# TritonDataCenter/containerpilot

Hardware: NVIDIA H100
Metric: events/sec through Bus.Publish (deliveries/s = 32-byte records landed in subscriber mailboxes) (higher is better)
Workload: dtype u8

## Files before the change

containerpilot_b200/_native.py:

```python
from __future__ import annotations

import ctypes as C
import os

import numpy as np

HERE = os.path.dirname(os.path.abspath(__file__))
LIB_PATH = os.environ.get("CPBUS_LIB") or os.path.join(HERE, "libcpbus.so")

N_CODES = 17
MASK_ALL = 0x0001FFFF
TARGET_ALL = 0xFFFFFFFF
F_TICK, F_UNICAST = 0x1, 0x2
CFG_LOSSLESS, CFG_DIGEST, CFG_SPARSE_TICKS, CFG_SPARSE_RECORDS = 0x1, 0x2, 0x4, 0x8
CFG_DROP_MISSED_TICKS = 0x10
STORE_AUTO, STORE_V4, STORE_V8, STORE_BULK = 0, 1, 2, 3

OK, EINVAL, ENOMEM, ECUDA, EAGAIN, ENOSPC, ENOENT, ECLOSED, ENODEV, EORDER, ETIMEDOUT = 0, -1, -2, -3, -4, -5, -6, -7, -8, -9, -10
PUT_STAMP, PUT_RAW, PUT_NOWAIT = 0, 1, 2
EPHEMERAL_BIT, EPHEMERAL_SLOTS = 0x80000000, 65536
DUE_CLOCK, DUE_ARM, DUE_ONESHOT, DUE_DISARM, DUE_UNSUB, DUE_LAUNCH = 0, 1, 2, 3, 4, 5
DUE_CATCHUP = 6


# ... 83 lines not shown
    "cpbus_stream_set_timeout": (C.c_int, [C.c_void_p, C.c_uint32]),
    "cpbus_stream_close": (C.c_int, [C.c_void_p]),
    "cpbus_shared_alloc": (C.c_int, [C.c_void_p, C.c_size_t, _P(C.c_void_p), C.c_char_p]),
    "cpbus_shared_open": (C.c_int, [C.c_void_p, C.c_char_p, _P(C.c_void_p)]),
    "cpbus_shared_close": (C.c_int, [C.c_void_p, C.c_void_p]),
    "cpbus_drain": (C.c_int, [C.c_void_p, C.c_uint32, C.c_void_p, C.c_size_t, _P(C.c_size_t), _P(C.c_uint64)]),
    "cpbus_drain_many": (C.c_int, [C.c_void_p, C.c_uint32, C.c_uint32, C.c_void_p, C.c_size_t, C.c_void_p, C.c_void_p, _P(C.c_size_t)]),
    "cpbus_drain_ready": (C.c_int, [C.c_void_p, C.c_uint32, C.c_uint32, C.c_uint32, C.c_void_p, C.c_size_t, C.c_void_p,
                                    C.c_size_t, _P(C.c_size_t), _P(C.c_size_t), _P(C.c_uint32)]),
    "cpbus_lagging": (C.c_int, [C.c_void_p, C.c_uint32, C.c_uint32, C.c_uint32, C.c_uint32, C.c_void_p, C.c_size_t,
                                _P(C.c_size_t), _P(C.c_uint32), _P(LagSummary)]),
    "cpbus_blockers": (C.c_int, [C.c_void_p, C.c_void_p, C.c_size_t, _P(C.c_size_t)]),
    "cpbus_stream_blockers": (C.c_int, [C.c_void_p, C.c_void_p, C.c_size_t, _P(C.c_size_t)]),
    "cpbus_consume_all": (C.c_int, [C.c_void_p]),
    "cpbus_peek_window": (C.c_int, [C.c_void_p, C.c_uint32, C.c_void_p, C.c_size_t, _P(C.c_size_t)]),
    "cpbus_digest": (C.c_int, [C.c_void_p, C.c_uint32, C.c_uint32, C.c_void_p]),
    "cpbus_digest_fold": (C.c_int, [C.c_void_p, C.c_uint32, C.c_uint32, _P(C.c_uint64 * 4)]),
    "cpbus_digest_fold_begin": (C.c_int, [C.c_void_p, C.c_uint32, C.c_uint32, _P(C.c_uint32)]),
    "cpbus_digest_fold_end": (C.c_int, [C.c_void_p, C.c_uint32, _P(C.c_uint64 * 4)]),
    "cpbus_step_result_begin": (C.c_int, [C.c_void_p, _P(C.c_uint32)]),
    "cpbus_step_result_end": (C.c_int, [C.c_void_p, C.c_uint32, _P(C.c_uint64 * 4)]),
    "cpbus_debug_events": (C.c_int, [C.c_void_p, C.c_void_p, C.c_size_t, _P(C.c_size_t)]),
    "cpbus_stats": (C.c_int, [C.c_void_p, _P(Stats)]),
    "cpbus_publish_counts": (C.c_int, [C.c_void_p, C.c_void_p, C.c_size_t, _P(C.c_size_t)]),
    "cpbus_device_ptrs": (C.c_int, [C.c_void_p, _P(C.c_void_p), _P(C.c_void_p)]),
    "cpbus_code_name": (C.c_char_p, [C.c_int]),
    "cpbus_code_from_string": (C.c_int, [C.c_char_p]),
    "cpbus_strerror": (C.c_char_p, [C.c_int]),
    "cpbus_last_cuda_error": (C.c_char_p, []),
    "cpbus_abi_version": (C.c_uint32, []),
    "cpbus_split_plan": (C.c_int, [C.c_void_p, C.c_size_t, C.c_uint32, C.c_uint64, C.c_uint64, C.c_uint64, C.c_void_p, C.c_void_p, C.c_size_t, _P(C.c_size_t)]),
    "cpbus_mask_order": (C.c_size_t, [C.c_void_p, C.c_void_p, C.c_uint32, C.c_uint32, C.c_uint32, C.c_int, C.c_void_p]),
    "cpbus_due_trace": (C.c_int, [C.c_void_p, C.c_size_t, C.c_uint32, C.c_uint32, C.c_void_p, C.c_size_t, _P(C.c_size_t)]),
    "cpbus_sparse_plan": (C.c_int, [C.c_void_p, C.c_void_p, C.c_uint32, C.c_void_p, C.c_void_p, C.c_uint32, C.c_void_p,
                                    C.c_size_t, C.c_void_p, C.c_size_t, C.c_uint32, C.c_size_t, C.c_size_t, C.c_void_p,
                                    C.c_size_t, C.c_void_p, C.c_size_t, _P(C.c_size_t), _P(C.c_size_t)]),
    "cpbus_record_hash": (C.c_uint64, [_P(Event)]),
    "cpbus_digest_multiplier": (C.c_uint64, []),
}
GROUP_CALLS = ("intern", "intern_ephemeral", "source", "subscribe", "subscribe_many", "subscribe_pairs", "subscribe_pairs_many",
               "unsubscribe", "set_mask", "timer_add", "timer_add_many", "timer_cancel", "publish", "send", "advance", "flush",
               "sync", "drain", "drain_ready", "lagging", "blockers", "consume_all", "peek_window", "digest", "digest_fold",
               "debug_events", "stats", "publish_counts")
SYMBOLS["cpbus_group_create"] = (C.c_int, [_P(Config), C.c_void_p, C.c_uint32, _P(C.c_void_p)])
SYMBOLS["cpbus_group_destroy"] = (C.c_int, [C.c_void_p])
SYMBOLS.update({f"cpbus_group_{name}": SYMBOLS[f"cpbus_{name}"] for name in GROUP_CALLS})
# ... 34 lines not shown
```

containerpilot_b200/csrc/cpbus.cu:

```cuda
#include "cpbus_kernels.cuh"

#include <algorithm>
#include <chrono>
#include <cstdio>
#include <cstdlib>
#include <cstring>
#include <deque>
#include <map>
#include <mutex>
#include <new>
#include <string>
#include <thread>
#include <unordered_map>
#include <vector>

using namespace cpbus_dev;

namespace {

thread_local char g_cuda_err[256] = "";

#define CK(call)                                                                                   \
  do {                                                                                             \
    cudaError_t e_ = (call);                                                                       \
// ... 362 lines not shown
  static constexpr int kStage = 8;
  static constexpr int kDevSlots = 64, kDevEpoch = 16;
  cpbus_event* d_stage = nullptr;
  cudaEvent_t epoch_done[kDevSlots / kDevEpoch] = {};
  uint32_t dev_slot = 0;
  cpbus_event* h_batch[kStage] = {};
  cudaEvent_t h2d_done[kStage] = {};
  cudaStream_t copy_stream = nullptr;
  cudaStream_t result_stream = nullptr;
  DevResultSlot* d_result = nullptr;
  DevResultSlot* h_result = nullptr;
  cudaEvent_t result_done[8] = {};
  uint32_t result_next = 0;
  DevStats* h_stats = nullptr;
  unsigned long long* h_fold = nullptr;
  int cur = 0;

  std::vector<uint32_t> h_mask;
  std::vector<uint8_t> h_active;
  std::vector<uint8_t> h_npairs;
  uint2* d_pairs = nullptr;
  uint32_t n_paired = 0;
  uint32_t* d_order = nullptr;
  uint32_t n_order = 0, n_filtered = 0;
  bool order_dirty = true;
  uint32_t n_next = 0, n_active = 0;

  uint64_t room_lb = 0;

  bool sparse = false, sparse_records = false;
  DueIndex due;
  std::vector<uint32_t> due_slots;
  SubIndex rec_index;
  std::vector<cpbus_plan_entry> plan;
  std::vector<uint32_t> plan_idx;
  std::vector<uint64_t> plan_pairs;
  unsigned char* h_plan = nullptr; unsigned char* d_plan = nullptr; size_t plan_bytes_cap = 0;
  cudaEvent_t plan_done = nullptr;
  cudaEvent_t records_done = nullptr;
  std::vector<uint32_t> catchup_slots;
  uint32_t* d_catchup = nullptr; size_t catchup_cap = 0;

  std::unordered_map<std::string, uint32_t> intern;
  std::vector<std::string> sources;
  size_t intern_bytes = 0;
  struct EphSlot { std::string s; uint32_t gen = 0; bool live = false; };
// ... 103 lines not shown
    for (size_t k = 1; k < count.size(); k++) count[k] += count[k - 1];
    const size_t base = order.size();
    order.resize(base + count.back());
    for (uint32_t i = lo; i < hi; i++) if (!active || active[i]) order[base + count[masks[i] & CPBUS_MASK_ALL]++] = i;
    if (heavy_first) {
      const size_t nb = order.size() - base;
      uint32_t pc_count[34] = {};
      for (size_t k = 0; k < nb; k++) pc_count[32 - __builtin_popcount(masks[order[base + k]] & CPBUS_MASK_ALL) + 1]++;
      for (int k = 1; k < 34; k++) pc_count[k] += pc_count[k - 1];
      tmp.resize(nb);
      for (size_t k = 0; k < nb; k++) tmp[pc_count[32 - __builtin_popcount(masks[order[base + k]] & CPBUS_MASK_ALL)]++] = order[base + k];
      std::copy(tmp.begin(), tmp.end(), order.begin() + base);
    }
  }
}

int rebuild_order(cpbus* b) {
  std::vector<uint32_t> order;
  static_assert(sizeof(b->h_active[0]) == 1, "h_active is a byte vector");
  mask_order(b->h_mask.data(), reinterpret_cast<const uint8_t*>(b->h_active.data()), b->n_next, b->R, b->order_block, true, order);
  b->n_order = (uint32_t)order.size();
  if (b->n_order) {
    CK(cudaMemcpyAsync(b->d_order, order.data(), (size_t)b->n_order * 4, cudaMemcpyHostToDevice, b->stream));
    CK(cudaStreamSynchronize(b->stream));
  }
  b->order_dirty = false;
  return CPBUS_OK;
}

constexpr int kFanoutMaxSmem = 200 * 1024;

enum { kLaunchPlain = 0, kLaunchFollow = 1, kLaunchRound = 2 };

template <int STORE, bool TIMERS, bool DIGEST, bool ORDERED, bool PAIRS = false>
int launch_fanout_t(cpbus* b, const FanoutParams& p, uint32_t grid, size_t smem, int kind) {
  static bool attr_done[3][64] = {};
  void (*kernel)(FanoutParams) = kind == kLaunchRound  ? fanout_round_kernel<STORE, TIMERS, DIGEST, ORDERED, PAIRS>
                               : kind == kLaunchFollow ? fanout_follow_kernel<STORE, TIMERS, DIGEST, ORDERED, PAIRS>
                                                       : fanout_kernel<STORE, TIMERS, DIGEST, ORDERED, PAIRS>;
  const int dev = b->device & 63;
  if (!attr_done[kind][dev]) {
    CK(cudaFuncSetAttribute(kernel, cudaFuncAttributeMaxDynamicSharedMemorySize, kFanoutMaxSmem));
    attr_done[kind][dev] = true;
  }
  cudaLaunchConfig_t cfg{};
  cfg.gridDim = dim3(grid); cfg.blockDim = dim3(kThreads); cfg.dynamicSmemBytes = smem; cfg.stream = b->stream;
// ... 90 lines not shown
  if (follow) {
    p.follow_clock = b->d_follow_clock; p.follow_rec = sa->follow_rec; p.follow_window = max_window(b);
    p.follow_from_host = sa->follow_from_host ? 1u : 0u;
  }
  p.prefetch_src = o.pf_src; p.prefetch_dst = o.pf_dst; p.prefetch_n = o.pf_n;
  p.batch_dep = o.batch_dep ? 1u : 0u; p.n_ev = n;
  p.n_subs = b->n_next; p.ring_cap = b->R; p.K = b->K; p.sub_base = b->cfg.sub_id_base;
  p.use_digest = b->use_digest; p.lossless = b->lossless; p.timers_on = b->n_timers > 0 && b->K > 0;
  p.smem_cap = (n + 31u) & ~31u;
  const size_t hot_bytes = (size_t)b->n_next * (sizeof(SubCtl) + (p.timers_on ? b->K * sizeof(DevTimer) : 0));
  p.hints = b->hints >= 0 ? (uint32_t)b->hints : (hot_bytes <= (64u << 20) ? 1u : 0u);
  const uint32_t need = (b->n_next + kWarpsPerCta - 1) / kWarpsPerCta;
  uint32_t grid = b->cfg.grid_ctas ? std::max(1u, std::min(b->cfg.grid_ctas, need)) : 0u;
  int rc;
  const bool pairs_on = b->n_paired > 0 && b->d_pairs;
  p.pairs = pairs_on ? b->d_pairs : nullptr;
  size_t smem = fanout_smem_bytes(p.smem_cap) + (pairs_on ? kPairFilterBytes : 0);
  if (!pairs_on && !p.timers_on && b->n_filtered > 0) {
    if (b->order_dirty) { const int rc_order = rebuild_order(b); if (rc_order) return rc_order; }
    if (b->n_order) {
      const uint32_t scale = std::max(1u, (p.n_ev + 128u) / 256u);
      uint32_t spw = b->subs_per_warp ? std::min(32u, b->subs_per_warp)
                                      : std::max(4u, std::min(16u / scale, b->n_order / (20480u * scale)));
      p.order = b->d_order; p.n_order = b->n_order; p.spw = spw;
      const uint32_t warps = (b->n_order + spw - 1) / spw;
      grid = std::max(1u, (warps + kWarpsPerCta - 1) / kWarpsPerCta);
    }
  }
  if (pairs_on && !b->cfg.grid_ctas) {
    const uint32_t blocks = (b->n_next + 31u) / 32u;
    grid = std::max(1u, std::min((blocks + kWarpsPerCta - 1) / kWarpsPerCta, (uint32_t)b->sm_count * 16u));
  }
  if (!pairs_on && !p.order) {
    uint32_t spw = b->subs_per_warp;
    if (grid) spw = std::max(1u, (need + grid - 1) / grid);
    else if (!spw) {
      const uint32_t scale = std::max(1u, (p.n_ev + 128u) / 256u);
      const uint32_t cap = std::max(1u, 16u / scale);
      spw = std::max(1u, std::min(cap, (need + (uint32_t)b->sm_count * 7 * scale) / ((uint32_t)b->sm_count * 14 * scale)));
    }
    p.spw = spw;
    grid = std::max(1u, (need + spw - 1) / spw);
    const size_t off = fanout_stage_off(p.smem_cap);
    const size_t per_sub = sizeof(SubCtl) + (p.timers_on ? (size_t)b->K * sizeof(DevTimer) : 0);
    const size_t min_round = (size_t)kWarpsPerCta * per_sub;
    const size_t ctas = std::max<size_t>(1, std::min<size_t>(kCtasPerSm, b->smem_per_sm / (off + min_round + b->smem_reserved)));
    const size_t room = std::min<size_t>(kFanoutMaxSmem, b->smem_per_sm / ctas - b->smem_reserved) - off;
    p.stage_subs = std::max<uint32_t>(kWarpsPerCta, (uint32_t)std::min<size_t>((size_t)kWarpsPerCta * spw, room / per_sub) & ~7u);
    smem = off + p.stage_subs * per_sub;
// ... 613 lines not shown
  int rc = CPBUS_OK;
  auto fail = [&](int code) { cpbus_destroy(b); return code; };
  if (cfg->device >= 0) b->device = cfg->device;
  else if (cudaGetDevice(&b->device) != cudaSuccess) return fail(CPBUS_ECUDA);
  if (b->device >= ndev) return fail(CPBUS_EINVAL);
  if ((rc = dev_guard(b))) return fail(rc);
  cudaDeviceProp prop{};
  if (cudaGetDeviceProperties(&prop, b->device) == cudaSuccess) {
    b->sm_count = prop.multiProcessorCount;
    b->smem_per_sm = prop.sharedMemPerMultiprocessor; b->smem_reserved = prop.reservedSharedMemPerBlock;
  }
  if (cfg->stream) b->stream = (cudaStream_t)cfg->stream;
  else {
    if (cudaStreamCreateWithFlags(&b->stream, cudaStreamNonBlocking) != cudaSuccess) return fail(CPBUS_ECUDA);
    b->own_stream = true;
  }
  const size_t N = b->N;
#define ALLOC(ptr, bytes)                                                                     \
  if (cudaMalloc((void**)&(ptr), (bytes)) != cudaSuccess) {                                   \
    snprintf(g_cuda_err, sizeof(g_cuda_err), "cudaMalloc(%zu) failed", (size_t)(bytes));     \
    return fail(CPBUS_ENOMEM);                                                                \
  }
  ALLOC(b->d_ring, N * R * sizeof(cpbus_event));
  ALLOC(b->d_ctl, N * sizeof(SubCtl)); ALLOC(b->d_order, N * 4);
  if (K) ALLOC(b->d_timers, N * K * sizeof(DevTimer));
  ALLOC(b->d_stats, sizeof(DevStats)); ALLOC(b->d_fold, 32 * cpbus::kFoldSlots); ALLOC(b->d_pow, kPowTableLen * 8);
  ALLOC(b->d_desc, 2 * ((fanout_desc_bytes(2048) + 255) & ~(size_t)255)); ALLOC(b->d_desc_ready, 256);
  if (cudaMemsetAsync(b->d_desc_ready, 0, 256, b->stream) != cudaSuccess) return fail(CPBUS_ECUDA);
  if (cudaStreamCreateWithFlags(&b->copy_stream, cudaStreamNonBlocking) != cudaSuccess) return fail(CPBUS_ECUDA);
  if (cudaStreamCreateWithFlags(&b->result_stream, cudaStreamNonBlocking) != cudaSuccess) return fail(CPBUS_ECUDA);
  if (cudaEventCreateWithFlags(&b->launched, cudaEventDisableTiming) != cudaSuccess) return fail(CPBUS_ECUDA);
  if (b->sparse && (cudaEventCreateWithFlags(&b->plan_done, cudaEventDisableTiming) != cudaSuccess ||
                    cudaEventCreateWithFlags(&b->records_done, cudaEventDisableTiming) != cudaSuccess))
    return fail(CPBUS_ECUDA);
  ALLOC(b->d_stage, (size_t)cpbus::kDevSlots * B * sizeof(cpbus_event));
  for (int i = 0; i < cpbus::kDevSlots / cpbus::kDevEpoch; i++)
    if (cudaEventCreateWithFlags(&b->epoch_done[i], cudaEventDisableTiming) != cudaSuccess) return fail(CPBUS_ECUDA);
  for (int i = 0; i < cpbus::kStage; i++) {
    if (cudaMallocHost((void**)&b->h_batch[i], (size_t)B * sizeof(cpbus_event)) != cudaSuccess) return fail(CPBUS_ENOMEM);
    if (cudaEventCreateWithFlags(&b->h2d_done[i], cudaEventDisableTiming) != cudaSuccess) return fail(CPBUS_ECUDA);
  }
  ALLOC(b->d_batch_local, (size_t)B * sizeof(cpbus_event));
  if (b->lossless) {
    ALLOC(b->d_admit_batch, (size_t)B * sizeof(cpbus_event));
    ALLOC(b->d_round, sizeof(RoundDev));
    RoundDev init{};
    init.room_full = R;
// ... 40 lines not shown
        cudaStreamSynchronize(b->stream) != cudaSuccess) return fail(CPBUS_ECUDA);
  }
  b->h_mask.assign(N, 0);
  b->h_active.assign(N, 0);
  if (b->sparse_records) b->rec_index.init(N, 2 * std::max<size_t>(32, N / 1024));
  else if (b->sparse) b->rec_index.slot.assign(N, UINT32_MAX);
  b->intern.emplace(std::string(), 0u);
  b->sources.emplace_back();
  *out = b;
  return CPBUS_OK;
} CPBUS_CATCH

int cpbus_destroy(cpbus_t* b) try {
  if (!b) return CPBUS_EINVAL;
  follow_resolve(b);
  cudaSetDevice(b->device);
  if (b->stream) cudaStreamSynchronize(b->stream);
  while (!b->streams.empty()) cpbus_stream_close(b->streams.back());
  if (b->h_follow) cudaFreeHost(b->h_follow);
  cudaFree(b->d_follow_clock);
  if (b->h_round) cudaFreeHost(b->h_round);
  cudaFree(b->d_round);
  if (b->follow_done) cudaEventDestroy(b->follow_done);
  cudaFree(b->d_ring); cudaFree(b->d_ctl); cudaFree(b->d_order); cudaFree(b->d_pairs);
  cudaFree(b->d_timers); cudaFree(b->d_stats); cudaFree(b->d_fold); cudaFree(b->d_pow); cudaFree(b->d_desc); cudaFree(b->d_desc_ready);
  if (b->copy_stream) cudaStreamSynchronize(b->copy_stream);
  if (b->result_stream) { cudaStreamSynchronize(b->result_stream); cudaStreamDestroy(b->result_stream); }
  for (int i = 0; i < cpbus::kStage; i++) {
    if (b->h_batch[i]) cudaFreeHost(b->h_batch[i]);
    if (b->h2d_done[i]) cudaEventDestroy(b->h2d_done[i]);
  }
  cudaFree(b->d_stage);
  for (int i = 0; i < cpbus::kDevSlots / cpbus::kDevEpoch; i++) if (b->epoch_done[i]) cudaEventDestroy(b->epoch_done[i]);
  if (b->copy_stream) cudaStreamDestroy(b->copy_stream);
  if (b->launched) cudaEventDestroy(b->launched);
  if (b->plan_done) cudaEventDestroy(b->plan_done);
  if (b->records_done) cudaEventDestroy(b->records_done);
  cudaFree(b->d_plan);
  if (b->h_plan) cudaFreeHost(b->h_plan);
  cudaFree(b->d_catchup);
  cudaFree(b->d_drain);cudaFree(b->d_drain_idx);
  cudaFree(b->d_ready_lb); cudaFree(b->d_ready); cudaFree(b->d_ready_slot);
  if (b->h_ready_hdr) cudaFreeHost(b->h_ready_hdr);
  cudaFree(b->d_lag_lb);
  if (b->h_lag_hdr) cudaFreeHost(b->h_lag_hdr);
  if (b->h_block) cudaFreeHost(b->h_block);
  if (b->h_lag) cudaFreeHost(b->h_lag);
// ... 1343 lines not shown
  CK(cudaMemsetAsync(&b->d_stats->overwritten, 0, sizeof(unsigned long long), b->stream));
  if (!b->lossless && b->n_next) {
    const uint32_t threads = 256, grid = std::min<uint32_t>((b->n_next + threads - 1) / threads, (uint32_t)b->sm_count * 4);
    overwritten_kernel<<<grid, threads, 0, b->stream>>>(b->d_ctl, b->n_next, b->R, &b->d_stats->overwritten);
    CK(cudaGetLastError());
  }
  CK(cudaMemcpyAsync(b->h_stats, b->d_stats, sizeof(DevStats), cudaMemcpyDeviceToHost, b->stream));
  CK(cudaMemcpyAsync(b->h_acct->by_code, b->d_acct->by_code, sizeof(b->h_acct->by_code), cudaMemcpyDeviceToHost, b->stream));
  CK(cudaStreamSynchronize(b->stream));
  retire_oneshots(b, b->last_watermark);
  b->st.deliveries = b->st.ticks = 0;
  b->st.overwritten = b->h_stats->overwritten;
  for (int i = 0; i < kStatSlots; i++) { b->st.deliveries += b->h_stats->slot[i].deliveries; b->st.ticks += b->h_stats->slot[i].ticks; }
  b->st.n_subs = b->n_active; b->st.n_timers = b->n_timers; b->st.now_ns = b->now;
  b->st.intern_entries = b->sources.size(); b->st.intern_bytes = b->intern_bytes;
  b->st.ephemeral_live = b->eph_live; b->st.ephemeral_recycled = b->eph_recycled;
  *out = b->st;
  out->publishes = b->publishes;
  for (int c = 0; c < CPBUS_N_CODES; c++)
    out->published_by_code[c] = b->published_by_code[c] + b->h_acct->by_code[c];
  return CPBUS_OK;
} CPBUS_CATCH

int cpbus_publish_counts(cpbus_t* b, cpbus_pair_count* out, size_t cap, size_t* n) try {
  if (!b || !n || (!out && cap)) return CPBUS_EINVAL;
  std::lock_guard<std::mutex> g(b->mu);
  int rc = enter(b); if (rc) return rc;
  std::vector<unsigned long long> keys, cnts;
  if (b->launch_seq) {
    keys.resize(kAcctPairSlots); cnts.resize(kAcctPairSlots);
    CK(cudaMemcpyAsync(keys.data(), b->d_acct->pair_key, sizeof(unsigned long long) * kAcctPairSlots, cudaMemcpyDeviceToHost, b->stream));
    CK(cudaMemcpyAsync(cnts.data(), b->d_acct->pair_cnt, sizeof(unsigned long long) * kAcctPairSlots, cudaMemcpyDeviceToHost, b->stream));
    CK(cudaStreamSynchronize(b->stream));
  }
  pair_counts(b, keys.data(), cnts.data(), keys.size(), out, cap, n);
  return CPBUS_OK;
} CPBUS_CATCH

int cpbus_device_ptrs(cpbus_t* b, void** ring, void** ctl) try {
  if (!b) return CPBUS_EINVAL;
  if (ring) *ring = b->d_ring;
  if (ctl) *ctl = b->d_ctl;
  return CPBUS_OK;
} CPBUS_CATCH

static uint32_t group_shard_of(const cpbus_group* g, uint32_t index) {
// ... 441 lines not shown
```

containerpilot_b200/csrc/cpbus_fanout_body.cuh:

```cuda
  constexpr bool STAGED = !ORDERED && !PAIRS;
  extern __shared__ __align__(128) unsigned char smem[];
  const uint32_t cap = p.smem_cap;
  cpbus_event* s_batch = reinterpret_cast<cpbus_event*>(smem);
  uint64_t* s_rhash = reinterpret_cast<uint64_t*>(smem + (size_t)cap * 32);
  uint2* s_meta = reinterpret_cast<uint2*>(smem + (size_t)cap * 40);
  uint64_t* s_q = reinterpret_cast<uint64_t*>(smem + (size_t)cap * 48);
  uint32_t* s_dsum = reinterpret_cast<uint32_t*>(s_q + cap + 2);
  uint32_t* s_present = s_dsum + 40;
  uint64_t* s_pow = s_q + cap + 2 + 20 + (PAIRS ? kPairFilterWords / 2 : 0);
  BatchSummary* s_sum = reinterpret_cast<BatchSummary*>(s_pow + cap + 66);
  uint32_t* s_tick = reinterpret_cast<uint32_t*>(s_sum + 1);
  const uint4* s_ctl4 = reinterpret_cast<const uint4*>(smem + fanout_stage_off(cap));
  const uint4* s_tim4 = s_ctl4 + 2u * p.stage_subs;

  const int tid = threadIdx.x, lane = tid & 31, warp = tid >> 5;
  uint32_t n = FOLLOW ? 0u : p.n_ev;
  uint64_t w_follow = 0;
  unsigned long long round_ack = 0;

  if (p.batch_dep) asm volatile("griddepcontrol.wait;" ::: "memory");
  const bool stream = p.staged == 2u;
  const uint32_t pf_slot = stream ? (uint32_t)(p.stream_seq % kStreamPrefetch) : 0u;
  uint32_t pos = ORDERED ? (blockIdx.x * kWarpsPerCta + warp) * p.spw : 0u;
  uint32_t my_ids = 0;
// ... 239 lines not shown
    __syncthreads();
#pragma unroll
    for (int r = 0; r < 8; r++) { const uint32_t q = tid + r * kThreads; if (q < 2u * n) v[r] = sq[q]; }
    __syncthreads();
#pragma unroll
    for (int r = 0; r < 8; r++) { const uint32_t q = tid + r * kThreads; if (q < 2u * n) sq[(q & 1u) * hi_off + (q >> 1)] = v[r]; }
    __syncthreads();
  }
  auto ev_ts = [&](uint32_t i) -> uint64_t {
    return PLANAR ? reinterpret_cast<const uint64_t*>(reinterpret_cast<const uint4*>(s_batch) + i)[1] : s_batch[i].ts_ns;
  };
  auto ev_code_src = [&](uint32_t i) -> uint2 {
    return PLANAR ? reinterpret_cast<const uint2*>(reinterpret_cast<const uint4*>(s_batch) + hi_off + i)[0] : make_uint2(s_batch[i].code, s_batch[i].source_id);
  };
  const bool aborted = s_sum->abort_launch != 0;
  const uint32_t K = p.K, J = K ? 32u / K : 32u;
  const uint32_t tk_slot = lane / J, tk_j = lane % J;
  const bool timers_on = TIMERS && p.timers_on && K;
  const uint32_t wstride = gridDim.x * kWarpsPerCta;
  uint32_t pos_end = (aborted || !ORDERED) ? 0u : min(pos + p.spw, p.n_order);
  const uint32_t pos_step = ORDERED ? 1u : kWarpsPerCta;
  const uint32_t pos0 = pos;
  uint32_t s = ORDERED ? __shfl_sync(0xffffffffu, my_ids, 0) : pos;
  if (!p.batch_dep) asm volatile("griddepcontrol.wait;" ::: "memory");
  asm volatile("griddepcontrol.launch_dependents;");
  const uint32_t rng_first = blockIdx.x * kWarpsPerCta * p.spw, rng_end = min(rng_first + kWarpsPerCta * p.spw, p.n_subs);
  auto stage_round = [&](uint32_t first) {
    if (!STAGED || tid != 0 || aborted || first >= rng_end) return;
    const uint32_t rn = min(p.stage_subs, rng_end - first);
    asm volatile("fence.proxy.async.shared::cta;" ::: "memory");
    const uint32_t tim_bytes = timers_on ? rn * K * (uint32_t)sizeof(DevTimer) : 0u;
    mbar_expect_tx(&s_sum->mbar_state, rn * (uint32_t)sizeof(SubCtl) + tim_bytes);
    bulk_g2s_hint(const_cast<uint4*>(s_ctl4), p.ctl + first, rn * (uint32_t)sizeof(SubCtl), &s_sum->mbar_state, keep);
    if (tim_bytes) bulk_g2s_hint(const_cast<uint4*>(s_tim4), p.timers + (size_t)first * K, tim_bytes, &s_sum->mbar_state, keep);
  };
  uint4 ca = make_uint4(0, 0, 0, 0), cb = ca, ta = ca;
  if (ORDERED && pos < pos_end) ld_sector(p.ctl + s, ca, cb, keep);
  const uint32_t present = s_dsum[0];
  const bool has_unicast = s_dsum[1] != 0;
  bool bulk_pending = false;
  uint32_t tri_blk = blockIdx.x * kWarpsPerCta + warp, tri_base = 0, tri_live = 0;
  uint4 tri_a = make_uint4(0, 0, 0, 0), tri_b = tri_a;
  uint32_t rnd_first = rng_first, rnd_phase = 0;
  for (;;) {
  if constexpr (STAGED) {
    if (aborted || rnd_first >= rng_end) break;
// ... 191 lines not shown
        copy_record_pairs<PLANAR>(s4, hi_off, ring, (uint32_t)tail, Rm, c0 + lane, out, c0 + lane < n);
      }
      if (!cold_early && TIMERS && tk_slot < nslots) {
        const uint4 cold = tim_half(1);
        tk_src = cold.x; tk_fired = cold.y;
      }
      if (tk_valid) {
        const uint32_t out = tk_pos + tk_rank;
        const uint64_t w0 = (uint64_t)tk_fired + tk_j, w1 = tk_due;
        const uint64_t w2 = (uint64_t)CPBUS_TIMER_EXPIRED | ((uint64_t)tk_src << 32);
        const uint64_t w3 = (uint64_t)gid | ((uint64_t)CPBUS_F_TICK << 32);
        const uint4 a = make_uint4((uint32_t)w0, (uint32_t)(w0 >> 32), (uint32_t)w1, (uint32_t)(w1 >> 32));
        const uint4 b = make_uint4((uint32_t)w2, (uint32_t)(w2 >> 32), (uint32_t)w3, (uint32_t)(w3 >> 32));
        st_v8(ring + (((uint32_t)tail + out) & Rm), a, b);
        if (DIGEST) {
          const uint32_t prev = tk_rank ? my_tick[tk_rank - 1] : 0u;
          dsum = (s_q[tk_pos] - s_q[prev]) * s_pow[n_ticks - tk_rank] + record_hash_words(w0, w1, w2, w3) * s_pow[k - 1 - out];
          if (tk_rank == n_ticks - 1) dsum += s_q[n] - s_q[tk_pos];
        }
      }
      if (DIGEST) dsum = warp_sum64(dsum);
      __syncwarp();
    } else if (!(PAIRS && pair_live) && !has_unicast && n_ticks == 0) {
      if constexpr (!TIMERS) {
        uint16_t* my_idx = reinterpret_cast<uint16_t*>(my_tick);
        const bool reuse = ORDERED && (m & CPBUS_MASK_ALL) == run_mask;
        if (!reuse) {
          uint32_t base = 0;
          const uint32_t nchunks = (n + 31) >> 5;
          for (uint32_t c0 = 0; c0 < nchunks; c0 += 4) {
            uint32_t cbit[4];
#pragma unroll
            for (uint32_t u = 0; u < 4; u++) {
              const uint32_t i = (c0 + u) * 32 + lane;
              cbit[u] = i < n ? s_meta[i].x : 0u;
            }
#pragma unroll
            for (uint32_t u = 0; u < 4; u++) {
              const bool match = (m & cbit[u]) != 0;
              const uint32_t w = __ballot_sync(0xffffffffu, match);
              if (match) my_idx[base + __popc(w & ((1u << lane) - 1u))] = (uint16_t)((c0 + u) * 32 + lane);
              base += __popc(w);
            }
          }
          run_k = base;
          __syncwarp();
        }
// ... 146 lines not shown
      atomicAdd(&s_sum->acc_deliv, k);
      if (DIGEST) {
        const uint32_t f = (uint32_t)nd ^ (uint32_t)(nd >> 32);
        atomicAdd(&s_sum->acc_dig_lo, f & 0xFFFFu);
        atomicAdd(&s_sum->acc_dig_hi, f >> 16);
      }
      if (TIMERS && n_ticks) atomicAdd(&s_sum->acc_ticks, n_ticks);
    }
  }

  if constexpr (ORDERED) break;
  if constexpr (STAGED) {
    __syncthreads();
    rnd_first += p.stage_subs;
  }
  }
  if (STORE == CPBUS_STORE_BULK && bulk_pending && lane == 0)
    asm volatile("cp.async.bulk.wait_group 0;" ::: "memory");
  __syncthreads();
  if (tid == 0) {
    DevStatSlot* st = &p.stats->slot[blockIdx.x % kStatSlots];
    if (s_sum->acc_deliv) atomicAdd(&st->deliveries, (unsigned long long)s_sum->acc_deliv);
    if (s_sum->acc_ticks) atomicAdd(&st->ticks, (unsigned long long)s_sum->acc_ticks);
    DevResultSlot* rs = &p.result[blockIdx.x % kResultSub];
    if (s_sum->acc_deliv) atomicAdd(&rs->deliveries, (unsigned long long)s_sum->acc_deliv);
    if (s_sum->acc_ticks) atomicAdd(&rs->ticks, (unsigned long long)s_sum->acc_ticks);
    if (s_sum->acc_dig_lo | s_sum->acc_dig_hi) atomicAdd(&rs->digest_sum, (unsigned long long)s_sum->acc_dig_lo + ((unsigned long long)s_sum->acc_dig_hi << 16));
    if (blockIdx.x == 0) atomicAdd(&rs->launch_seq, p.launch_seq);
  }
  if (blockIdx.x == 0 && p.acct && !aborted) {
    if (tid < CPBUS_N_CODES && tid != CPBUS_METRIC && s_dsum[2 + tid]) atomicAdd(&p.acct->by_code[tid], (unsigned long long)s_dsum[2 + tid]);
    for (uint32_t i = tid; i < n; i += kThreads) {
      if (s_meta[i].y != CPBUS_TARGET_ALL) continue;
      const uint2 cs = ev_code_src(i);
      const uint32_t code = cs.x;
      if (code == CPBUS_METRIC || code >= CPBUS_N_CODES) continue;
      const unsigned long long key = (((unsigned long long)code << 32) | cs.y) + 1ull;
      uint32_t slot = pair_key_hash(code, cs.y) & (kAcctPairSlots - 1u);
      bool placed = false;
      for (int probe = 0; probe < 32 && !placed; probe++, slot = (slot + 1u) & (kAcctPairSlots - 1u)) {
        const unsigned long long old = atomicCAS(&p.acct->pair_key[slot], 0ull, key);
        if (old == 0ull || old == key) { atomicAdd(&p.acct->pair_cnt[slot], 1ull); placed = true; }
      }
      if (!placed) atomicAdd(&p.acct->pair_overflow, 1ull);
    }
    if (tid == 0) {
// ... 52 lines not shown
```

containerpilot_b200/csrc/cpbus_kernels.cuh:

```cuda
#pragma once
#include <cstdint>
#include <cuda_runtime.h>

#include "../../include/cpbus.h"

namespace cpbus_dev {

constexpr int kWarpsPerCta = 8;
constexpr int kThreads = kWarpsPerCta * 32;
constexpr int kCtasPerSm = 4;
constexpr uint32_t kActiveBit = 0x80000000u;
constexpr int kTimerHintShift = 24;
constexpr uint32_t kPairBit = 0x10000000u;
constexpr uint32_t kPairNone = 0xFFFFFFFFu;
constexpr uint32_t kCodeOutOfRange = CPBUS_N_CODES;
static_assert(kCodeOutOfRange < (uint32_t)kTimerHintShift,"the out-of-range bit must lie between the code mask and the mask word's bookkeeping bits");
constexpr uint32_t kPairFilterWords = 1024;
constexpr uint32_t kPairFilterBytes = kPairFilterWords * 4;
__host__ __device__ inline uint32_t pair_key_hash(uint32_t code, uint32_t source_id) {
  uint32_t x = (source_id ^ (code << 27)) * 0x9E3779B1u;
  x ^= x >> 15; x *= 0x85EBCA77u; x ^= x >> 13;
  return x;
}
constexpr uint64_t kDigestP = 0x9E3779B97F4A7C15ull;
constexpr uint32_t kPowTableLen = 2048 + 65 + 7;

struct __align__(32) DevTimer {
  uint64_t next_due;
  uint64_t period;
  uint32_t source_id;
  uint32_t fired;
  uint32_t pad[2];
};
constexpr uint64_t kTimerIdle = ~0ull;

constexpr int kStatSlots = 256;
struct __align__(32) DevStatSlot { unsigned long long deliveries, ticks, pad[2]; };
struct DevStats {
  DevStatSlot slot[kStatSlots];
  unsigned long long admit_overflow, overwritten;
  unsigned long long admit_max_used;
  unsigned long long admit_deficit;
};

constexpr uint32_t kAcctPairSlots = 1u << 19;
constexpr int kAcctDbgRing = 64, kAcctDbgKeep = 10;
struct __align__(32) DevDbgTail {
  unsigned long long launch_seq;
  uint32_t n_broadcast, n_kept;
  cpbus_event ev[kAcctDbgKeep];
  uint32_t pad[4];
};
struct DevPubAcct {
  unsigned long long by_code[32];
  unsigned long long pair_overflow, pad[3];
  DevDbgTail tail[kAcctDbgRing];
  unsigned long long pair_key[kAcctPairSlots];
  unsigned long long pair_cnt[kAcctPairSlots];
};

// ... 94 lines not shown
  uint64_t w_now;
  uint32_t n_ev, n_subs, ring_cap, K, sub_base;
  uint32_t use_digest, lossless, timers_on;
  uint32_t smem_cap;
  uint32_t hints;
  const uint2* pairs;
  const StreamHdr* stream_hdr;
  unsigned long long* stream_ack;
  unsigned long long stream_seq;
  const StreamHdr* stream_next_hdr;
  uint32_t stream_off;
  uint32_t stream_final;
  unsigned long long* pf_state;
  cpbus_event* pf_buf;
  uint32_t pf_stride;
  uint32_t spin_us;
  unsigned int* err_word;
  DevPubAcct* acct;
  unsigned long long* follow_clock;
  FollowRec* follow_rec;
  uint64_t follow_window;
  uint32_t follow_from_host;
  const RoundDev* round;
};

__host__ __device__ inline uint64_t record_hash_words(uint64_t w0, uint64_t w1, uint64_t w2, uint64_t w3) {
  const uint64_t K0 = 0x9E3779B97F4A7C15ull, K1 = 0xBF58476D1CE4E5B9ull,
                 K2 = 0x94D049BB133111EBull, K3 = 0xD6E8FEB86659FD93ull,
                 K4 = 0xA0761D6478BD642Full;
  uint64_t x = (w0 + K4) * K0; x ^= x >> 32;
  x = (x + w1) * K1; x ^= x >> 32;
  x = (x + w2) * K2; x ^= x >> 32;
  x = (x + w3) * K3; x ^= x >> 29;
  return x;
}

__host__ __device__ inline uint64_t pow_p(uint32_t e) {
  uint64_t r = 1, b = kDigestP;
  while (e) { if (e & 1u) r *= b; b *= b; e >>= 1; }
  return r;
}

#ifdef __CUDACC__
__device__ __forceinline__ uint32_t smem_u32(const void* p) { return (uint32_t)__cvta_generic_to_shared(p); }
__device__ __forceinline__ uint64_t shfl64(uint64_t v, int src) {
  uint32_t lo = __shfl_sync(0xffffffffu, (uint32_t)v, src);
// ... 93 lines not shown
      : "memory");
}

struct BatchSummary {
  uint64_t mbar;
  uint64_t mbar_desc;
  uint64_t mbar_state;
  uint32_t acc_deliv, acc_ticks, acc_pad[2];
  uint32_t acc_dig_lo, acc_dig_hi;
  uint32_t stream_local;
  uint32_t own_desc;
  uint32_t abort_launch;
  uint32_t pf_ok;
  uint64_t red[kWarpsPerCta];
};

__host__ __device__ inline size_t fanout_desc_bytes(uint32_t cap) { return (size_t)24 * cap + 16 + 160 + kPairFilterBytes; }

__host__ __device__ inline size_t fanout_smem_bytes(uint32_t cap) {
  const size_t scratch = (cap / 2u > 32u ? cap / 2u : 32u) * sizeof(uint32_t);
  return (size_t)cap * 56 + 16 + 160 + (size_t)(cap + 66) * 8 + sizeof(BatchSummary) + kWarpsPerCta * scratch + 128;
}
__host__ __device__ inline size_t fanout_stage_off(uint32_t cap) { return (fanout_smem_bytes(cap) + 127) & ~(size_t)127; }

template <int STORE, bool TIMERS, bool DIGEST, bool ORDERED, bool PAIRS = false>
__global__ void __launch_bounds__(kThreads, kCtasPerSm) fanout_kernel(const FanoutParams p) {
  constexpr bool FOLLOW = false, ROUND = false;
#include "cpbus_fanout_body.cuh"
}
template <int STORE, bool TIMERS, bool DIGEST, bool ORDERED, bool PAIRS = false>
__global__ void __launch_bounds__(kThreads, kCtasPerSm) fanout_follow_kernel(const FanoutParams p) {
  constexpr bool FOLLOW = true, ROUND = false;
#include "cpbus_fanout_body.cuh"
}
template <int STORE, bool TIMERS, bool DIGEST, bool ORDERED, bool PAIRS = false>
__global__ void __launch_bounds__(kThreads, kCtasPerSm) fanout_round_kernel(const FanoutParams p) {
  constexpr bool FOLLOW = true, ROUND = true;
#include "cpbus_fanout_body.cuh"
}

__device__ __forceinline__ void admit_body(const cpbus_event* batch, uint32_t n_ev, uint64_t w_now, const SubCtl* ctl,
                                           const DevTimer* timers, uint32_t n_subs, uint32_t ring_cap, uint32_t K,
                                           uint32_t sub_base, uint32_t timers_on, DevStats* stats, const uint2* pairs) {
  __shared__ uint32_t hist[32];
  __shared__ uint32_t s_uni;
  __shared__ unsigned long long s_max;
// ... 792 lines not shown
```

include/cpbus.h:

```cpp
#ifndef CPBUS_H
#define CPBUS_H

#include <stddef.h>
#include <stdint.h>

#ifdef __cplusplus
extern "C" {
#endif

enum {
  CPBUS_NONE = 0, CPBUS_EXIT_SUCCESS, CPBUS_EXIT_FAILED, CPBUS_STOPPING,
  CPBUS_STOPPED, CPBUS_STATUS_HEALTHY, CPBUS_STATUS_UNHEALTHY,
  CPBUS_STATUS_CHANGED, CPBUS_TIMER_EXPIRED, CPBUS_ENTER_MAINTENANCE,
  CPBUS_EXIT_MAINTENANCE, CPBUS_ERROR, CPBUS_QUIT, CPBUS_METRIC,
  CPBUS_STARTUP, CPBUS_SHUTDOWN, CPBUS_SIGNAL,
  CPBUS_N_CODES
};

#define CPBUS_MASK_ALL 0x0001FFFFu

typedef struct cpbus_pair { uint32_t code, source_id; } cpbus_pair;
#define CPBUS_MAX_PAIRS 16

#define CPBUS_TARGET_ALL 0xFFFFFFFFu
// ... 153 lines not shown
} cpbus_lag;
typedef struct cpbus_lag_summary {
  uint64_t active;
  uint64_t lagging;
  uint64_t backlog_total, backlog_max, lost_total;
  uint64_t hist[33];
} cpbus_lag_summary;
int cpbus_lagging(cpbus_t* bus, uint32_t first_sub, uint32_t n, uint32_t start_sub, uint32_t min_backlog,
                  cpbus_lag* out, size_t cap, size_t* n_out, uint32_t* next_sub, cpbus_lag_summary* sum);
int cpbus_blockers(cpbus_t* bus, uint32_t* out, size_t cap, size_t* n);
int cpbus_stream_blockers(cpbus_stream_t* st, uint32_t* out, size_t cap, size_t* n);
int cpbus_consume_all(cpbus_t* bus);
int cpbus_peek_window(cpbus_t* bus, uint32_t sub_id, cpbus_event* out, size_t cap, size_t* n);
int cpbus_digest(cpbus_t* bus, uint32_t first_sub, uint32_t n, cpbus_digest_t* out);
int cpbus_digest_fold(cpbus_t* bus, uint32_t first_sub, uint32_t n, uint64_t out[4]);
int cpbus_digest_fold_begin(cpbus_t* bus, uint32_t first_sub, uint32_t n, uint32_t* ticket);
int cpbus_digest_fold_end(cpbus_t* bus, uint32_t ticket, uint64_t out[4]);

int cpbus_step_result_begin(cpbus_t* bus, uint32_t* ticket);
int cpbus_step_result_end(cpbus_t* bus, uint32_t ticket, uint64_t out[4]);

int cpbus_debug_events(cpbus_t* bus, cpbus_event* out, size_t cap, size_t* n);
int cpbus_stats(cpbus_t* bus, cpbus_stats_t* out);
typedef struct cpbus_pair_count { uint32_t code, source_id; uint64_t count; } cpbus_pair_count;
int cpbus_publish_counts(cpbus_t* bus, cpbus_pair_count* out, size_t cap, size_t* n);
int cpbus_device_ptrs(cpbus_t* bus, void** ring, void** ctl);

typedef struct cpbus_group cpbus_group_t;
int cpbus_group_create(const cpbus_config* cfg, const int32_t* devices, uint32_t n_devices, cpbus_group_t** out);
int cpbus_group_destroy(cpbus_group_t* g);
int cpbus_group_intern(cpbus_group_t* g, const char* s, size_t len, uint32_t* source_id);
int cpbus_group_intern_ephemeral(cpbus_group_t* g, const char* s, size_t len, uint32_t* source_id);
int cpbus_group_source(cpbus_group_t* g, uint32_t source_id, char* out, size_t cap, size_t* len);
int cpbus_group_subscribe(cpbus_group_t* g, uint32_t code_mask, uint32_t* sub_id);
int cpbus_group_subscribe_many(cpbus_group_t* g, const uint32_t* code_masks, uint32_t n, uint32_t* first_sub_id);
int cpbus_group_subscribe_pairs(cpbus_group_t* g, uint32_t code_mask, const cpbus_pair* pairs, uint32_t n_pairs, uint32_t* sub_id);
int cpbus_group_subscribe_pairs_many(cpbus_group_t* g, const uint32_t* code_masks, const cpbus_pair* pairs,
                                     const uint32_t* n_pairs, uint32_t n, uint32_t* first_sub_id);
int cpbus_group_unsubscribe(cpbus_group_t* g, uint32_t sub_id);
int cpbus_group_set_mask(cpbus_group_t* g, uint32_t sub_id, uint32_t code_mask);
int cpbus_group_timer_add(cpbus_group_t* g, uint32_t sub_id, uint64_t period_ns, uint32_t source_id, int oneshot, uint32_t* timer_id);
int cpbus_group_timer_add_many(cpbus_group_t* g, uint32_t first_sub, uint32_t n, uint64_t period_ns, const uint32_t* source_ids,
                               uint32_t source_id0, int oneshot);
int cpbus_group_timer_cancel(cpbus_group_t* g, uint32_t timer_id);
int cpbus_group_publish(cpbus_group_t* g, const cpbus_event* ev, size_t n);
int cpbus_group_send(cpbus_group_t* g, uint32_t sub_id, const cpbus_event* ev);
// ... 47 lines not shown
```

Baseline: 93.12 billion.

## Prebuild per-CTA filtered event images in shared memory for repeated subscriber masks

For the ordered fanout path, each CTA now finds the distinct partial-match subscriber masks in its range, using a new per-subscriber device mask array. For up to eight of them it compacts the matching batch records, with their digest, into a shared-memory image once. Mailboxes with those masks then copy the prebuilt image instead of filtering per subscriber, and mailboxes matching no present code skip work. The extra shared memory is sized from the SM budget, which may lower occupancy, and the setup adds several block-wide barriers. New counters and an API expose how many mailboxes took the image path versus the fallback.

```diff
diff --git a/containerpilot_b200/_native.py b/containerpilot_b200/_native.py
--- a/containerpilot_b200/_native.py
+++ b/containerpilot_b200/_native.py
@@ -129,6 +129,7 @@
     "cpbus_step_result_end": (C.c_int, [C.c_void_p, C.c_uint32, _P(C.c_uint64 * 4)]),
     "cpbus_debug_events": (C.c_int, [C.c_void_p, C.c_void_p, C.c_size_t, _P(C.c_size_t)]),
     "cpbus_stats": (C.c_int, [C.c_void_p, _P(Stats)]),
+    "cpbus_filter_paths": (C.c_int, [C.c_void_p, _P(C.c_uint64), _P(C.c_uint64)]),
     "cpbus_publish_counts": (C.c_int, [C.c_void_p, C.c_void_p, C.c_size_t, _P(C.c_size_t)]),
     "cpbus_device_ptrs": (C.c_int, [C.c_void_p, _P(C.c_void_p), _P(C.c_void_p)]),
     "cpbus_code_name": (C.c_char_p, [C.c_int]),
diff --git a/containerpilot_b200/csrc/cpbus.cu b/containerpilot_b200/csrc/cpbus.cu
--- a/containerpilot_b200/csrc/cpbus.cu
+++ b/containerpilot_b200/csrc/cpbus.cu
@@ -408,6 +408,7 @@
   uint2* d_pairs = nullptr;
   uint32_t n_paired = 0;
   uint32_t* d_order = nullptr;
+  uint32_t* d_order_mask = nullptr;
   uint32_t n_order = 0, n_filtered = 0;
   bool order_dirty = true;
   uint32_t n_next = 0, n_active = 0;
@@ -557,6 +558,9 @@
   b->n_order = (uint32_t)order.size();
   if (b->n_order) {
     CK(cudaMemcpyAsync(b->d_order, order.data(), (size_t)b->n_order * 4, cudaMemcpyHostToDevice, b->stream));
+    std::vector<uint32_t> order_mask(order.size());
+    for (size_t i = 0; i < order.size(); i++) order_mask[i] = b->h_mask[order[i]] & CPBUS_MASK_ALL;
+    CK(cudaMemcpyAsync(b->d_order_mask, order_mask.data(), (size_t)b->n_order * 4, cudaMemcpyHostToDevice, b->stream));
     CK(cudaStreamSynchronize(b->stream));
   }
   b->order_dirty = false;
@@ -693,9 +697,15 @@
       const uint32_t scale = std::max(1u, (p.n_ev + 128u) / 256u);
       uint32_t spw = b->subs_per_warp ? std::min(32u, b->subs_per_warp)
                                       : std::max(4u, std::min(16u / scale, b->n_order / (20480u * scale)));
-      p.order = b->d_order; p.n_order = b->n_order; p.spw = spw;
+      p.order = b->d_order; p.order_mask = b->d_order_mask; p.n_order = b->n_order; p.spw = spw;
       const uint32_t warps = (b->n_order + spw - 1) / spw;
       grid = std::max(1u, (warps + kWarpsPerCta - 1) / kWarpsPerCta);
+      const size_t base = fanout_smem_bytes(p.smem_cap);
+      const size_t ctas = std::max<size_t>(1, std::min<size_t>(kCtasPerSm, b->smem_per_sm / (base + sizeof(ImgHdr) + b->smem_reserved)));
+      const size_t room = std::min<size_t>(kFanoutMaxSmem, b->smem_per_sm / ctas - b->smem_reserved);
+      const size_t hdr = (sizeof(ImgHdr) + 127) & ~(size_t)127;
+      p.img_bytes = (uint32_t)(room > base + hdr ? (room - base) & ~(size_t)127 : hdr);
+      smem = base + p.img_bytes;
     }
   }
   if (pairs_on && !b->cfg.grid_ctas) {
@@ -1355,7 +1365,7 @@
     return fail(CPBUS_ENOMEM);                                                                \
   }
   ALLOC(b->d_ring, N * R * sizeof(cpbus_event));
-  ALLOC(b->d_ctl, N * sizeof(SubCtl)); ALLOC(b->d_order, N * 4);
+  ALLOC(b->d_ctl, N * sizeof(SubCtl)); ALLOC(b->d_order, N * 4); ALLOC(b->d_order_mask, N * 4);
   if (K) ALLOC(b->d_timers, N * K * sizeof(DevTimer));
   ALLOC(b->d_stats, sizeof(DevStats)); ALLOC(b->d_fold, 32 * cpbus::kFoldSlots); ALLOC(b->d_pow, kPowTableLen * 8);
   ALLOC(b->d_desc, 2 * ((fanout_desc_bytes(2048) + 255) & ~(size_t)255)); ALLOC(b->d_desc_ready, 256);
@@ -1442,7 +1452,7 @@
   if (b->h_round) cudaFreeHost(b->h_round);
   cudaFree(b->d_round);
   if (b->follow_done) cudaEventDestroy(b->follow_done);
-  cudaFree(b->d_ring); cudaFree(b->d_ctl); cudaFree(b->d_order); cudaFree(b->d_pairs);
+  cudaFree(b->d_ring); cudaFree(b->d_ctl); cudaFree(b->d_order); cudaFree(b->d_order_mask); cudaFree(b->d_pairs);
   cudaFree(b->d_timers); cudaFree(b->d_stats); cudaFree(b->d_fold); cudaFree(b->d_pow); cudaFree(b->d_desc); cudaFree(b->d_desc_ready);
   if (b->copy_stream) cudaStreamSynchronize(b->copy_stream);
   if (b->result_stream) { cudaStreamSynchronize(b->result_stream); cudaStreamDestroy(b->result_stream); }
@@ -2832,6 +2842,18 @@
   return CPBUS_OK;
 } CPBUS_CATCH
 
+int cpbus_filter_paths(cpbus_t* b, uint64_t* image_mailboxes, uint64_t* fallback_mailboxes) try {
+  if (!b || !image_mailboxes || !fallback_mailboxes) return CPBUS_EINVAL;
+  std::lock_guard<std::mutex> g(b->mu);
+  int rc = enter(b); if (rc) return rc;
+  CK(cudaMemcpyAsync(b->h_stats->slot, b->d_stats->slot, sizeof(b->h_stats->slot), cudaMemcpyDeviceToHost, b->stream));
+  CK(cudaStreamSynchronize(b->stream));
+  uint64_t img = 0, fb = 0;
+  for (int i = 0; i < kStatSlots; i++) { img += b->h_stats->slot[i].img_mailboxes; fb += b->h_stats->slot[i].fallback_mailboxes; }
+  *image_mailboxes = img; *fallback_mailboxes = fb;
+  return CPBUS_OK;
+} CPBUS_CATCH
+
 int cpbus_publish_counts(cpbus_t* b, cpbus_pair_count* out, size_t cap, size_t* n) try {
   if (!b || !n || (!out && cap)) return CPBUS_EINVAL;
   std::lock_guard<std::mutex> g(b->mu);
diff --git a/containerpilot_b200/csrc/cpbus_fanout_body.cuh b/containerpilot_b200/csrc/cpbus_fanout_body.cuh
--- a/containerpilot_b200/csrc/cpbus_fanout_body.cuh
+++ b/containerpilot_b200/csrc/cpbus_fanout_body.cuh
@@ -285,6 +285,95 @@
   const uint32_t pos_step = ORDERED ? 1u : kWarpsPerCta;
   const uint32_t pos0 = pos;
   uint32_t s = ORDERED ? __shfl_sync(0xffffffffu, my_ids, 0) : pos;
+  if constexpr (ORDERED) {
+    const uint32_t present = s_dsum[0];
+    const uint32_t sw8 = kWarpsPerCta * max(32u, cap / 2u);
+    ImgHdr* ih = reinterpret_cast<ImgHdr*>(reinterpret_cast<unsigned char*>(s_tick + sw8) + p.img_bytes - sizeof(ImgHdr));
+    const bool img_on = !aborted && n && n <= kImgMaxEvents && s_dsum[1] == 0;
+    if (tid == 0) { ih->n_img = 0; s_sum->acc_pad[0] = 0; s_sum->acc_pad[1] = 0; }
+    if (img_on) {
+      const uint32_t cta_first = blockIdx.x * kWarpsPerCta * p.spw;
+      const uint32_t cta_n = min(kWarpsPerCta * p.spw, p.n_order - min(p.n_order, cta_first));
+      uint32_t mk = 0;
+      if ((uint32_t)tid < cta_n) {
+        const uint32_t mm = __ldg(p.order_mask + cta_first + tid) & CPBUS_MASK_ALL;
+        if ((mm & present) != present && (mm & present) != 0) mk = mm;
+      }
+      s_tick[tid] = mk;
+      __syncthreads();
+      const bool head = mk && (tid == 0 || s_tick[tid - 1] != mk);
+      const uint32_t hb = __ballot_sync(0xffffffffu, head);
+      if (lane == 0) ih->wcnt[warp] = __popc(hb);
+      __syncthreads();
+      uint32_t r = __popc(hb & ((1u << lane) - 1u));
+      for (int w = 0; w < warp; w++) r += ih->wcnt[w];
+      if (head && r < kImgSlots) ih->slot[r].mask = mk;
+      __syncthreads();
+      if (warp == 0) {
+        uint32_t heads = 0;
+        for (int w = 0; w < kWarpsPerCta; w++) heads += ih->wcnt[w];
+        const uint32_t ns = min(heads, kImgSlots);
+        uint32_t k = 0;
+        if ((uint32_t)lane < ns)
+          for (uint32_t b = ih->slot[lane].mask & present; b; b &= b - 1u) k += s_dsum[2 + __ffs(b) - 1];
+        uint32_t cum = k;
+#pragma unroll
+        for (int o = 1; o < 32; o <<= 1) {
+          const uint32_t t = __shfl_up_sync(0xffffffffu, cum, o);
+          if (lane >= o) cum += t;
+        }
+        const uint32_t above = (p.img_bytes - (uint32_t)sizeof(ImgHdr)) / 32u;
+        const bool ok = (uint32_t)lane < ns && cum <= above;
+        const uint32_t first = sw8 / 8u + cum - k;
+        if (ok) { ih->slot[lane].k = k; ih->slot[lane].off = 2u * first; ih->slot[lane].dig = 0ull; }
+        const uint32_t n_ok = __popc(__ballot_sync(0xffffffffu, ok));
+        if (lane == 0) ih->n_img = n_ok;
+      }
+      __syncthreads();
+      const uint32_t n_img = ih->n_img, nchunks = (n + 31u) >> 5;
+      for (uint32_t j = 0; j < n_img; j++) {
+        const uint32_t mj = ih->slot[j].mask;
+        for (uint32_t c = warp; c < nchunks; c += kWarpsPerCta) {
+          const uint32_t i = c * 32u + lane;
+          const uint32_t w = __ballot_sync(0xffffffffu, i < n && (mj & s_meta[i].x) != 0);
+          if (lane == 0) ih->cnt[j][c] = __popc(w);
+        }
+      }
+      __syncthreads();
+      if ((uint32_t)warp < n_img) {
+        const uint32_t v = (uint32_t)lane < nchunks ? ih->cnt[warp][lane] : 0u;
+        uint32_t incl = v;
+#pragma unroll
+        for (int o = 1; o < 32; o <<= 1) {
+          const uint32_t t = __shfl_up_sync(0xffffffffu, incl, o);
+          if (lane >= o) incl += t;
+        }
+        if ((uint32_t)lane < nchunks) ih->cnt[warp][lane] = incl - v;
+      }
+      __syncthreads();
+      uint4* img = reinterpret_cast<uint4*>(s_tick);
+      const uint4* sb = reinterpret_cast<const uint4*>(s_batch);
+      for (uint32_t j = 0; j < n_img; j++) {
+        const uint32_t mj = ih->slot[j].mask, kj = ih->slot[j].k, off = ih->slot[j].off;
+        uint64_t h = 0;
+        for (uint32_t c = warp; c < nchunks; c += kWarpsPerCta) {
+          const uint32_t i = c * 32u + lane;
+          const bool match = i < n && (mj & s_meta[i].x) != 0;
+          const uint32_t w = __ballot_sync(0xffffffffu, match);
+          if (match) {
+            const uint32_t o = ih->cnt[j][c] + __popc(w & ((1u << lane) - 1u));
+            img[off + 2u * o] = sb[2u * i]; img[off + 2u * o + 1u] = sb[2u * i + 1u];
+            if (DIGEST) h += s_rhash[i] * s_pow[kj - 1u - o];
+          }
+        }
+        if (DIGEST) {
+          h = warp_sum64(h);
+          if (lane == 0 && h) atomicAdd(reinterpret_cast<unsigned long long*>(&ih->slot[j].dig), (unsigned long long)h);
+        }
+      }
+    }
+    __syncthreads();
+  }
   if (!p.batch_dep) asm volatile("griddepcontrol.wait;" ::: "memory");
   asm volatile("griddepcontrol.launch_dependents;");
   const uint32_t rng_first = blockIdx.x * kWarpsPerCta * p.spw, rng_end = min(rng_first + kWarpsPerCta * p.spw, p.n_subs);
@@ -522,7 +611,25 @@
       if (DIGEST) dsum = warp_sum64(dsum);
       __syncwarp();
     } else if (!(PAIRS && pair_live) && !has_unicast && n_ticks == 0) {
-      if constexpr (!TIMERS) {
+      uint32_t img_j = kImgSlots;
+      const ImgHdr* ih = nullptr;
+      if constexpr (ORDERED) {
+        ih = reinterpret_cast<const ImgHdr*>(reinterpret_cast<const unsigned char*>(s_tick + kWarpsPerCta * max(32u, cap / 2u)) +
+                                             p.img_bytes - sizeof(ImgHdr));
+        const uint32_t n_img = ih->n_img;
+        for (uint32_t j = 0; j < n_img; j++)
+          if (ih->slot[j].mask == (m & CPBUS_MASK_ALL)) { img_j = j; break; }
+      }
+      if (ORDERED && (m & present) == 0) {
+      } else if (ORDERED && img_j < kImgSlots) {
+        k = ih->slot[img_j].k;
+        const uint4* img = reinterpret_cast<const uint4*>(s_tick) + ih->slot[img_j].off;
+        for (uint32_t c0 = 0; c0 < k; c0 += 32)
+          copy_record_pairs<false>(img, 0u, ring, (uint32_t)tail, Rm, c0 + lane, c0 + lane, c0 + lane < k);
+        if (DIGEST) dsum = ih->slot[img_j].dig;
+        if (lane == 0) atomicAdd(&s_sum->acc_pad[0], 1u);
+      } else if constexpr (!TIMERS) {
+        if (ORDERED && lane == 0) atomicAdd(&s_sum->acc_pad[1], 1u);
         uint16_t* my_idx = reinterpret_cast<uint16_t*>(my_tick);
         const bool reuse = ORDERED && (m & CPBUS_MASK_ALL) == run_mask;
         if (!reuse) {
@@ -715,6 +822,8 @@
     DevStatSlot* st = &p.stats->slot[blockIdx.x % kStatSlots];
     if (s_sum->acc_deliv) atomicAdd(&st->deliveries, (unsigned long long)s_sum->acc_deliv);
     if (s_sum->acc_ticks) atomicAdd(&st->ticks, (unsigned long long)s_sum->acc_ticks);
+    if (ORDERED && s_sum->acc_pad[0]) atomicAdd(&st->img_mailboxes, (unsigned long long)s_sum->acc_pad[0]);
+    if (ORDERED && s_sum->acc_pad[1]) atomicAdd(&st->fallback_mailboxes, (unsigned long long)s_sum->acc_pad[1]);
     DevResultSlot* rs = &p.result[blockIdx.x % kResultSub];
     if (s_sum->acc_deliv) atomicAdd(&rs->deliveries, (unsigned long long)s_sum->acc_deliv);
     if (s_sum->acc_ticks) atomicAdd(&rs->ticks, (unsigned long long)s_sum->acc_ticks);
diff --git a/containerpilot_b200/csrc/cpbus_kernels.cuh b/containerpilot_b200/csrc/cpbus_kernels.cuh
--- a/containerpilot_b200/csrc/cpbus_kernels.cuh
+++ b/containerpilot_b200/csrc/cpbus_kernels.cuh
@@ -35,7 +35,7 @@
 constexpr uint64_t kTimerIdle = ~0ull;
 
 constexpr int kStatSlots = 256;
-struct __align__(32) DevStatSlot { unsigned long long deliveries, ticks, pad[2]; };
+struct __align__(32) DevStatSlot { unsigned long long deliveries, ticks, img_mailboxes, fallback_mailboxes; };
 struct DevStats {
   DevStatSlot slot[kStatSlots];
   unsigned long long admit_overflow, overwritten;
@@ -176,6 +176,8 @@
   uint64_t follow_window;
   uint32_t follow_from_host;
   const RoundDev* round;
+  uint32_t img_bytes;
+  const uint32_t* order_mask;
 };
 
 __host__ __device__ inline uint64_t record_hash_words(uint64_t w0, uint64_t w1, uint64_t w2, uint64_t w3) {
@@ -315,6 +317,19 @@
   return (size_t)cap * 56 + 16 + 160 + (size_t)(cap + 66) * 8 + sizeof(BatchSummary) + kWarpsPerCta * scratch + 128;
 }
 __host__ __device__ inline size_t fanout_stage_off(uint32_t cap) { return (fanout_smem_bytes(cap) + 127) & ~(size_t)127; }
+
+constexpr uint32_t kImgSlots = 8;
+constexpr uint32_t kImgMaxEvents = 1024;
+struct ImgSlot {
+  uint32_t mask, k, off, pad;
+  unsigned long long dig;
+  unsigned long long pad2;
+};
+struct ImgHdr {
+  ImgSlot slot[kImgSlots];
+  uint32_t n_img, pad0, wcnt[kWarpsPerCta], pad1[6];
+  uint32_t cnt[kImgSlots][32];
+};
 
 template <int STORE, bool TIMERS, bool DIGEST, bool ORDERED, bool PAIRS = false>
 __global__ void __launch_bounds__(kThreads, kCtasPerSm) fanout_kernel(const FanoutParams p) {
diff --git a/include/cpbus.h b/include/cpbus.h
--- a/include/cpbus.h
+++ b/include/cpbus.h
@@ -199,6 +199,7 @@
 
 int cpbus_debug_events(cpbus_t* bus, cpbus_event* out, size_t cap, size_t* n);
 int cpbus_stats(cpbus_t* bus, cpbus_stats_t* out);
+int cpbus_filter_paths(cpbus_t* bus, uint64_t* image_mailboxes, uint64_t* fallback_mailboxes);
 typedef struct cpbus_pair_count { uint32_t code, source_id; uint64_t count; } cpbus_pair_count;
 int cpbus_publish_counts(cpbus_t* bus, cpbus_pair_count* out, size_t cap, size_t* n);
 int cpbus_device_ptrs(cpbus_t* bus, void** ring, void** ctl);
```

Measured after the change: 93.13 billion (median of 6 runs). About the same (+0.0%).
